# alibaba-damo-academy/Inferix

Hardware: AMD Instinct MI355X
Metric: latent_frames_per_sec (higher is better)
Workload: dtype bf16; 1 GPU; Self-Forcing 480p bf16 (Wan2.1-T2V-1.3B causal DiT, 30 layers), block_size=3, 21 latent frames = 7 blocks x (4 denoise + 1 context) generator forwards, KV prefix 4680..32760 keys in the KV manager's cache (identity page map; page-table form: `streaming_steady`); `value` counts the generator calls (SURVEY 8d), the per-block VAE decode of config 2 is measured beside it under --full (`per_block_decod; batch=1, parallelism=single, layers=30, pair_forwards=True, pair_mode=streams

## Files before the change

### inferix_amd/csrc/ifx_attn.h

```cpp
#pragma once
#include "ifx_common.h"

#ifndef PP_TRACE
#define PP_TRACE 0
#endif
#ifndef PP_PD
#define PP_PD 2
#endif
#ifndef PP_DUAL_FR
#define PP_DUAL_FR 6
#endif

namespace ifx {

namespace pp {
constexpr int KT = 64;
constexpr int HD = 128;
constexpr int PD = PP_PD;
constexpr int RK = PD + 1, RV = PD + 2;
constexpr int K_OFF = 0;
constexpr int LDS_BYTES = (RK + RV) * 16384;
constexpr int LDS_SWP = 8 * 16384;
constexpr int LDS_ALLOC = PP_TRACE ? LDS_SWP + 24576 : (LDS_BYTES > LDS_SWP ? LDS_BYTES : LDS_SWP);
constexpr int LDS_DUAL = 5 * 16384;

constexpr int FR_PLAIN = 0;
constexpr int FR_FREE = 1;
constexpr int FR_SWP = 2;
constexpr int FR_SWP_DUAL = 3;
constexpr int FR_U4 = 5;
constexpr int FR_U6_DUAL = 6;
constexpr int FR_U4_PRE = 7;
constexpr int FR_U6_DUAL_PRE = 8;
}

__device__ __forceinline__ float attn_max3(float a, float b, float c) {
  float r;
  asm("v_max3_f32 %0, %1, %2, %3" : "=v"(r) : "v"(a), "v"(b), "v"(c));
  return r;
}
__device__ __forceinline__ float attn_half_max(float x) {
  float a = x, b = x, r;
  asm volatile("s_nop 1\n\tv_permlane32_swap_b32 %0, %1\n\ts_nop 1\n\tv_max_f32 %2, %0, %1" : "+v"(a), "+v"(b), "=v"(r));
  return r;
}

struct AttnArgsPP {
  const unsigned short* q;
  unsigned short* out;
  float* lse;
  const unsigned short* k;
  const unsigned short* v;
  KvAddr ka;
  int q_rows, heads, kv_start, kv_len, num_slots, q_tiles, per_xcd, total;
  int ldq, ldo;
  float scale, scale_log2;
  int splits, chunk_tiles;
  int kv_heads, q_per_kv;
  float* part_o;
  float* part_lse;
  int n_ranges;
  int rq0[8], rq1[8], rk0[8], rk1[8], rt0[9];
  unsigned ps_magic;
  unsigned* dbg_rescales;
};

struct AttnSchedule {
  int variant;
  int ng;
  int fr, fr_pre;
  int qt;
  int slots;
  int lds_bytes;
  bool pipelined() const { return fr >= pp::FR_SWP; }
};
constexpr AttnSchedule kAttnSchedules[6] = {
// ... 6 lines not shown
};
inline const AttnSchedule& attn_schedule(int variant) { return kAttnSchedules[variant - 2]; }

inline int attn_pick_variant(int variant, int q_rows, int heads) {
  if (variant >= 2 && variant <= 7) return variant;
  if (variant == 0 && q_rows > 0) {
    const int t256 = (q_rows + 255) / 256, t128 = (q_rows + 127) / 128;
    const float u256 = (float)q_rows / (256.f * t256), u128 = (float)q_rows / (128.f * t128);
    if (u128 > 1.1f * u256) return 6;
    if (heads > 0 && t256 * heads > 256) {
      const float c5 = (float)((t256 * heads + 255) / 256);
      const float c6 = (float)((t128 * heads + 511) / 512) / 0.953f;
      if (c6 < 0.95f * c5) return 6;
    }
  }
  return 7;
}

struct AttnLaunch {
  const unsigned short* q = nullptr;
  unsigned short* out = nullptr;
  float* lse = nullptr;
  const ifx_kv_view* kv = nullptr;
  int q_rows = 0, heads = 0;
  int ldq = 0, ldo = 0;
  int kv_start = 0, kv_len = 0;
  float scale = 0.f;
  int splits = 1;
  void* workspace = nullptr;
  int slot_base = 0, slot_cap = 0, *slots_used = nullptr;
  int n_ranges = 0;
  const int *q_ranges = nullptr, *k_ranges = nullptr;
};
int attn_plan(const AttnLaunch& L, int variant, AttnArgsPP& a, int& schedule, int& paged);
int launch_attn_pp(const AttnArgsPP& a, const AttnSchedule& s, int paged, bool write_partials, bool pre, dim3 grid,
                   hipStream_t stream);
int launch_attn_merge(const float* workspace, int slot_cap, int slots_used, unsigned short* out, float* lse, int q_rows,
                      int heads, hipStream_t stream, int ldo = 0);
size_t attn_pp_workspace_bytes(int q_rows, int heads, int splits);
int attn_pp_split_heuristic(int q_rows, int heads, int nkeys, int qt, int slots);

}
```

### inferix_amd/csrc/ifx_attn.hip

```cpp
#include <stdlib.h>
#include <type_traits>

#include "ifx_attn.h"

namespace ifx {

constexpr int QT = 128;
constexpr int KT = 64;
constexpr int HD = 128;

struct AttnArgs {
  const unsigned short* q;
  unsigned short* out;
  float* lse;
  const unsigned short* k;
  const unsigned short* v;
  KvAddr ka;
  int q_rows, heads, kv_start, kv_len, q_tiles, per_xcd, total;
  int ldq, ldo;
  float last_key_bias;
  int kv_heads, q_per_kv;
  float scale, scale_log2;
};

// ... 263 lines not shown
    }
  }
}

size_t attn_pp_workspace_bytes(int q_rows, int heads, int splits) {
  return splits <= 1 ? 0 : (size_t)splits * q_rows * heads * (128 + 1) * sizeof(float);
}

int attn_pp_split_heuristic(int q_rows, int heads, int nkeys, int qt, int slots) {
  const int tiles = ((q_rows + qt - 1) / qt) * heads;
  const int nt = (nkeys + pp::KT - 1) / pp::KT;
  if (tiles * 16 >= slots * 13 || nt < 16) return 1;
  int best = 1;
  float best_eff = (float)tiles / ((float)slots * ((tiles + slots - 1) / slots));
  static float base = -1.f;
  if (base < 0.f) {
    const char* e = getenv("IFX_ATTN_SPLIT_PENALTY");
    base = e ? (float)atof(e) : 0.01f;
  }
  const float part_mb = (float)q_rows * (float)heads * 516.f / 3.6e6f;
  const float pen = base * (part_mb > 1.f ? part_mb : 1.f);
  for (int s = 2; s <= 32 && s * 8 <= nt; ++s) {
    const int wg = tiles * s, rounds = (wg + slots - 1) / slots;
    const float eff = (float)wg / ((float)slots * rounds) * (1.f - pen * s);
    if (eff > best_eff + 1e-3f) best_eff = eff, best = s;
  }
  return best;
}

static KvAddr attn_kv_addr(const ifx_kv_view* kv) {
  return KvAddr{kv->page_table, kv->page_size, kv->page_table ? 0 : kv->seg_split, kv->page_table ? 0 : kv->seg_delta};
}

int attn_plan(const AttnLaunch& L, int variant, AttnArgsPP& a, int& schedule, int& paged) {
  const ifx_kv_view* kv = L.kv;
  const unsigned ps_magic = (kv->page_table && kv->page_size >= 2 && (long long)kv->num_slots * kv->page_size < (1ll << 32))
                                ? (unsigned)((1ull << 32) / (unsigned)kv->page_size) + 1u : 0u;
  paged = 0;
  if (kv->page_table != nullptr) paged = (kv->page_size >= 3 && ps_magic != 0) ? 1 : 2;
  else if (kv->seg_split > 0) paged = 1;
  int kv_start = L.kv_start, kv_len = L.kv_len, rows = L.q_rows, streams = L.heads;
  if (L.n_ranges > 0) {
    kv_start = 0x7fffffff, kv_len = 0, rows = 0;
    for (int i = 0; i < L.n_ranges; ++i) {
      kv_start = min(kv_start, L.k_ranges[2 * i]);
      kv_len = max(kv_len, L.k_ranges[2 * i + 1]);
      rows += L.q_ranges[2 * i + 1] - L.q_ranges[2 * i];
    }
    rows /= L.n_ranges;
    streams = L.heads * L.n_ranges;
  }
  schedule = attn_pick_variant(variant, rows, streams);
  if (L.n_ranges > 0 && !attn_schedule(schedule).pipelined()) schedule = 7;
  if (paged == 2) schedule = 2;
  const int QT = attn_schedule(schedule).qt;
  const bool partial = L.slot_cap > 0;
  a.q = L.q;
  a.out = partial ? nullptr : L.out;
  a.lse = L.lse;
  a.k = kv->k;
  a.v = kv->v;
  a.ka = attn_kv_addr(kv);
  a.q_rows = L.q_rows;
  a.heads = L.heads;
  a.ldq = L.ldq > 0 ? L.ldq : L.heads * 128;
  a.ldo = L.ldo > 0 ? L.ldo : L.heads * 128;
  a.kv_start = kv_start;
// ... 9 lines not shown
    const int* kr = L.k_ranges;
    int order[8];
    for (int i = 0; i < L.n_ranges; ++i) order[i] = i;
    for (int i = 1; i < L.n_ranges; ++i)
      for (int j = i; j > 0 && kr[2 * order[j] + 1] - kr[2 * order[j]] > kr[2 * order[j - 1] + 1] - kr[2 * order[j - 1]]; --j) {
        const int t = order[j];
        order[j] = order[j - 1];
        order[j - 1] = t;
      }
    a.rt0[0] = 0;
    for (int i = 0; i < L.n_ranges; ++i) {
      const int r = order[i];
      a.rq0[i] = L.q_ranges[2 * r], a.rq1[i] = L.q_ranges[2 * r + 1], a.rk0[i] = kr[2 * r], a.rk1[i] = kr[2 * r + 1];
      a.rt0[i + 1] = a.rt0[i] + (a.rq1[i] - a.rq0[i] + QT - 1) / QT;
    }
    a.q_tiles = a.rt0[L.n_ranges];
  }
  const int nt = (kv_len - kv_start + KT - 1) / KT;
  const int splits = max(1, min(L.n_ranges > 0 ? 1 : L.splits, nt));
  a.chunk_tiles = (nt + splits - 1) / splits;
  a.splits = (nt + a.chunk_tiles - 1) / a.chunk_tiles;
  if (partial && L.slot_base + a.splits > L.slot_cap) {
    set_error("ifx_attn_fwd_partial: slots [%d, %d) exceed the workspace's %d", L.slot_base, L.slot_base + a.splits, L.slot_cap);
    return IFX_EINVAL;
  }
  const int cap = partial ? L.slot_cap : a.splits;
  float* ws = (float*)L.workspace;
  a.part_o = ws ? ws + (size_t)L.slot_base * L.q_rows * L.heads * 128 : nullptr;
  a.part_lse = ws ? ws + (size_t)cap * L.q_rows * L.heads * 128 + (size_t)L.slot_base * L.heads * L.q_rows : nullptr;
  a.total = a.q_tiles * L.heads * a.splits;
  a.per_xcd = (a.total + 7) / 8;
  a.scale = L.scale > 0.f ? L.scale : 0.08838834764831845f;
  a.scale_log2 = a.scale * 1.4426950408889634f;
  if ((partial || a.splits > 1) && L.workspace == nullptr) {
    set_error("ifx_attn_fwd_paged_split: split / partial launches need a workspace");
    return IFX_EINVAL;
  }
  return IFX_OK;
}

}

using namespace ifx;

static int attn_check_view(const char* fn, const ifx_kv_view* kv, int heads,
                           const char* heads_text = "%s: heads %d is not a multiple of kv_heads %d") {
  IFX_REQUIRE(kv->head_dim == HD, "%s: head_dim %d not built (128 only)", fn, kv->head_dim);
  IFX_REQUIRE(heads > 0 && kv->kv_heads > 0 && heads % kv->kv_heads == 0, heads_text, fn, heads, kv->kv_heads);
  return IFX_OK;
}

static int attn_launch(const AttnLaunch& L, int variant, void* stream) {
  AttnArgsPP a;
  int schedule, paged;
  if (const int rc = attn_plan(L, variant, a, schedule, paged)) return rc;
  if (L.slots_used) *L.slots_used = a.splits;
  return launch_attn_pp(a, attn_schedule(schedule), paged, a.splits > 1 || L.slot_cap > 0, fabsf(a.scale_log2 - 1.0f) <= 2.5e-7f,
                        dim3(a.per_xcd * 8), (hipStream_t)stream);
}

static int attn_dispatch(const ifx_bf16* q, ifx_bf16* out, float* lse, const ifx_kv_view* kv, int32_t q_rows,
                         int32_t heads, int32_t kv_start, int32_t kv_len, float scale, int32_t splits, void* workspace,
                         int64_t workspace_bytes, void* stream, int32_t ldq = 0, int32_t ldo = 0, int32_t last_key_multiplicity = 1) {
  IFX_REQUIRE(q && out && kv && kv->k && kv->v, "ifx_attn_fwd_paged: null argument");
  if (ldq <= 0) ldq = heads * HD;
  if (ldo <= 0) ldo = heads * HD;
  IFX_REQUIRE(ldq >= heads * HD && ldo >= heads * HD && ldq % 8 == 0 && ldo % 8 == 0,
              "ifx_attn_fwd_paged: row strides (%d, %d) must be >= heads * 128 and multiples of 8", ldq, ldo);
  if (const int rc = attn_check_view("ifx_attn_fwd_paged", kv, heads)) return rc;
  IFX_REQUIRE(q_rows >= 0 && kv_start >= 0 && kv_len > kv_start && kv_len <= kv->num_slots,
              "ifx_attn_fwd_paged: key range [%d, %d) out of range (capacity %d)", kv_start, kv_len, kv->num_slots);
  IFX_REQUIRE(!kv->page_table || kv->page_size > 0, "ifx_attn_fwd_paged: page_size must be > 0");
  if (q_rows == 0) return IFX_OK;
  const int variant = attn_variant();
  if (last_key_multiplicity > 1) {
    IFX_REQUIRE(splits <= 1 && kv_len - kv_start <= 1024 && lse == nullptr,
                "ifx_attn_fwd_dedup: the multiplicity form is built for short key ranges (<= 1024 keys), unsplit, without LSE");
  }
  if (splits > 1)
    IFX_REQUIRE(workspace && workspace_bytes >= (int64_t)attn_pp_workspace_bytes(q_rows, heads, splits),
                "ifx_attn_fwd_paged_split: workspace of %lld B too small for %d splits (need %lld B)",
                (long long)workspace_bytes, splits, (long long)attn_pp_workspace_bytes(q_rows, heads, splits));
  if (splits > 1 || (last_key_multiplicity <= 1 && (variant >= 2 || (variant == 0 && q_rows >= 1024 && kv_len - kv_start > 1024)))) {
    AttnLaunch L;
    L.q = q, L.out = out, L.lse = lse, L.kv = kv;
    L.q_rows = q_rows, L.heads = heads, L.ldq = ldq, L.ldo = ldo;
    L.kv_start = kv_start, L.kv_len = kv_len, L.scale = scale;
    L.splits = splits > 1 ? splits : 1;
    L.workspace = splits > 1 ? workspace : nullptr;
    return attn_launch(L, variant, stream);
  }
// ... 137 lines not shown
```

### inferix_amd/csrc/ifx_attn_pp.hip

```cpp
#include <stdlib.h>
#include <type_traits>

#include "ifx_attn.h"
#include "ifx_launch.h"
#include "ifx_lds_dma.h"

#ifndef PP_ABLATE
#define PP_ABLATE 0
#endif
#ifndef PP_PACKED
#define PP_PACKED 1
#endif
#ifndef PP_PRIO
#define PP_PRIO 2
#endif
#ifndef PP_RING
#define PP_RING 6
#endif
#ifndef PP_SWP_RING
#define PP_SWP_RING 4
#endif
#ifndef PP_SWP_BALANCE
#define PP_SWP_BALANCE 1
#endif
// ... 13 lines not shown
namespace ifx {

typedef float pp_f32x2 __attribute__((ext_vector_type(2)));

__device__ __forceinline__ void pp_wait_tiles(int tiles) {
  if (tiles <= 0) asm volatile("s_waitcnt vmcnt(0)" ::: "memory");
  else if (tiles == 1) asm volatile("s_waitcnt vmcnt(4)" ::: "memory");
  else if (tiles == 2) asm volatile("s_waitcnt vmcnt(8)" ::: "memory");
  else if (tiles == 3) asm volatile("s_waitcnt vmcnt(12)" ::: "memory");
  else asm volatile("s_waitcnt vmcnt(16)" ::: "memory");
}

__device__ __forceinline__ void pp_page_range(const KvAddr& ka, unsigned ps_magic, int kk, int& lo, int& hi, int& off) {
  if (ka.pt == nullptr) {
    const bool up = ka.seg_split > 0 && kk >= ka.seg_split;
    lo = up ? ka.seg_split : 0;
    hi = (up || ka.seg_split <= 0) ? 0x7fffffff : ka.seg_split;
    off = up ? ka.seg_delta : 0;
    return;
  }
  const int pg = (int)__umulhi((unsigned)kk, ps_magic);
  int entry;
  asm volatile("s_load_dword %0, %1, %2\n\ts_waitcnt lgkmcnt(0)" : "=s"(entry) : "s"(ka.pt), "s"(pg * 4) : "memory");
  lo = pg * ka.ps;
  hi = lo + ka.ps;
  off = entry * ka.ps - lo;
}

template <int PAGED, bool SPLIT, int NG, int FR = 0>
__global__ __launch_bounds__(NG * 256, NG == 1 ? 2 : 1) void attn_fwd_pp_kernel(AttnArgsPP A) {
  using namespace pp;
  constexpr int QT = 128 * NG;
  extern __shared__ __attribute__((aligned(16))) unsigned char smem[];
  constexpr bool SWP = FR >= FR_SWP, DUAL = FR == FR_SWP_DUAL || FR == FR_U6_DUAL || FR == FR_U6_DUAL_PRE, U4 = FR == FR_U4 || FR == FR_U4_PRE,
                 U6 = FR == FR_U6_DUAL || FR == FR_U6_DUAL_PRE, CS = U4 || U6;
  constexpr bool PRE = FR == FR_U4_PRE || FR == FR_U6_DUAL_PRE;
  constexpr int PD = (FR == FR_SWP || U4) ? 3 : pp::PD, RK = DUAL ? 2 : (U4 ? 4 : (FR == FR_SWP ? 3 : pp::RK)),
                RV = DUAL ? 3 : (U4 ? 4 : (FR == FR_SWP ? 5 : pp::RV));
  constexpr int K_OFF = CS ? RV * 16384 : 0, V_OFF = CS ? 0 : RK * 16384;
  const int tid = threadIdx.x, lane = tid & 63;
  const int wave = __builtin_amdgcn_readfirstlane(tid >> 6);
  const int grp = (NG == 2 && PP_GROUP) ? (wave & 1) : (wave >> 2);
  const bool loader = wave < 8;
  const int hi = lane >> 5, l31 = lane & 31;

  const int xcd = blockIdx.x & 7, slot_i = blockIdx.x >> 3;
  const int wi = (!SPLIT && A.n_ranges > 0) ? (int)blockIdx.x : xcd * A.per_xcd + slot_i;
  if ((A.n_ranges == 0 && slot_i >= A.per_xcd) || wi >= A.total) return;
  int head, qt, sp = 0;
  if (SPLIT) {
    const int per_head = A.splits * A.q_tiles;
    head = wi / per_head;
    const int rem = wi - head * per_head;
    sp = rem / A.q_tiles;
    qt = rem - sp * A.q_tiles;
  } else if (A.n_ranges > 0) {
    qt = wi / A.heads;
    head = wi - qt * A.heads;
  } else {
    head = wi / A.q_tiles;
    qt = wi - head * A.q_tiles;
  }
  int kv_s = SPLIT ? A.kv_start + sp * A.chunk_tiles * KT : A.kv_start;
  int kv_e = SPLIT ? min(A.kv_len, kv_s + A.chunk_tiles * KT) : A.kv_len;
  int q_base = qt * QT, q_lim = A.q_rows;
  if (!SPLIT && A.n_ranges > 0) {
    int r = 0;
#pragma unroll
    for (int i = 1; i < 8; ++i)
      if (i < A.n_ranges && qt >= A.rt0[i]) r = i;
    q_base = A.rq0[r] + (qt - A.rt0[r]) * QT;
    q_lim = A.rq1[r];
    kv_s = A.rk0[r];
    kv_e = A.rk1[r];
  }
  const int row_stride = A.heads * HD;

  const int qrow = q_base + wave * 32 + l31;
  const int qrow_c = min(qrow, q_lim - 1);
  bf16x8 qf[8];
  {
    const unsigned short* qp = A.q + (size_t)qrow_c * A.ldq + head * HD + hi * 8;
#pragma unroll
    for (int ks = 0; ks < 8; ++ks) qf[ks] = *reinterpret_cast<const bf16x8*>(qp + ks * 16);
  }
  __builtin_amdgcn_s_waitcnt(0x0F70);
  const int row_bytes = A.kv_heads * HD * 2;
  const int kvh = head / A.q_per_kv;
  const int nkeys = kv_e - kv_s;
  const int NT = (nkeys + KT - 1) / KT;
  const unsigned valid_rows = PAGED ? (unsigned)A.num_slots : (unsigned)kv_e;
  const unsigned nrec = (valid_rows - 1) * (unsigned)row_bytes + 256u;
  const v4i krs = make_rsrc(A.k + kvh * HD, nrec);
  const v4i vrs = make_rsrc(A.v + kvh * HD, nrec);
  const unsigned lds00 = (unsigned)(unsigned long long)(lds_ptr_t)smem;
  const int last_key = kv_e - 1;
  int pc_lo = 0, pc_hi = 0, pc_off = 0;
  int lane_pack;
  {
    const int ln0 = __builtin_amdgcn_mbcnt_hi(~0u, __builtin_amdgcn_mbcnt_lo(~0u, 0u));
    const int pc0 = ln0 & 15, row0 = wave * 4 + (ln0 >> 4);
    lane_pack = (ln0 >> 4) * row_bytes + ((pc0 ^ (row0 & 15)) << 4) +
                (int)((unsigned)((((pc0 >> 2) ^ (row0 & 3)) << 2) | (pc0 & 3)) << 28);
  }
  auto issue_w = [&](int t, int wv, int what = 3) {
    unsigned lds0 = lds00 + wv * 1024;
    asm volatile("" : "+s"(lds0));
    int ln = 0;
    if constexpr (PAGED != 0) {
      ln = __builtin_amdgcn_mbcnt_hi(~0u, __builtin_amdgcn_mbcnt_lo(~0u, 0u));
      asm volatile("" : "+v"(ln));
    }
    int lp = lane_pack;
    asm volatile("" : "+v"(lp));
// ... 22 lines not shown
      } else {
#pragma unroll
        for (int r = 0; r < 2; ++r) {
          const int key0 = key00 + 32 * r;
          const int kk = min(key0, last_key);
          if (kk < pc_lo || kk >= pc_hi) pp_page_range(A.ka, A.ps_magic, kk, pc_lo, pc_hi, pc_off);
          int soff = (kk + pc_off) * row_bytes;
          int adj = 0;
          if (kk + 3 > last_key || kk + 3 >= pc_hi) {
            const int j = min(ln >> 4, last_key - kk);
            adj += ((ln >> 4) - j) * row_bytes;
            if (kk + min(3, last_key - kk) >= pc_hi) {
              int lo2, hi2, off2;
              pp_page_range(A.ka, A.ps_magic, pc_hi, lo2, hi2, off2);
              adj -= (kk + ((kk + j >= pc_hi) ? off2 : pc_off)) * row_bytes;
              soff = 0;
            }
          }
          if (what & 1) dma16(krs, kb + r * 8192, k_lane - adj, soff);
          if (what & 2) dma16(vrs, vb + r * 8192, v_lane - adj, soff);
        }
      }
    } else {
#pragma unroll
      for (int r = 0; r < 2; ++r) {
        const int key = min(kv_s + t * KT + wv * 4 + (ln >> 4) + 32 * r, last_key);
        const int delta = (A.ka.slot(key) - (ln >> 4)) * row_bytes;
        if (what & 1) dma16(krs, kb + r * 8192, k_lane + delta, 0);
        if (what & 2) dma16(vrs, vb + r * 8192, v_lane + delta, 0);
      }
    }
  };
  auto issue = [&](int t) { issue_w(t, wave); };

  f32x16 o[4];
#pragma unroll
  for (int d = 0; d < 4; ++d)
#pragma unroll
    for (int r = 0; r < 16; ++r) o[d][r] = 0.f;
  float m_run = -INFINITY, l_run = 0.f;
  const float c2 = PRE ? 1.0f : A.scale_log2;
  const int kswz = l31 & 15;
  const int vi = lane & 15, vg1 = (lane >> 4) & 1;
  const int v_rowq = vi >> 2;
  const int v_in = (vg1 << 5) | ((vi & 3) << 3);

  f32x16 s[2];
  bf16x8 pb[2][2];
  bf16x8 fA[4], fB[4];
  constexpr int RD = FR == FR_FREE ? PP_RING : 3, LA = RD - 1;
  bf16x8 fr[RD][2];
  pb[0][0] = pb[0][1] = pb[1][0] = pb[1][1] = bf16x8{};
  if (PP_ABLATE) {
#pragma unroll
    for (int i = 0; i < 4; ++i) fA[i] = fB[i] = bf16x8{};
    pb[0][0] = pb[0][1] = pb[1][0] = pb[1][1] = bf16x8{};
    s[0] = s[1] = f32x16{};
  }

  auto ldV = [&](bf16x8(&f)[4], const unsigned char* vb, int b, int s2) {
    if (PP_ABLATE & 4) return;
    const unsigned char* vr0 = vb + (32 * b + 16 * s2 + 4 * hi + v_rowq) * 256 + v_in;
    const unsigned char* vr1 = vr0 + 8 * 256;
#pragma unroll
    for (int d = 0; d < 4; ++d) {
      const int ch = (d ^ v_rowq) << 6;
// ... 746 lines not shown
        for (int e = 0; e < 4; ++e) acc[e] += w * v[u][e];
      }
    }
  }
  const float inv = 1.0f / den;
  u16x4 w4;
#pragma unroll
  for (int e = 0; e < 4; ++e) w4[e] = f2bf(acc[e] * inv);
  *reinterpret_cast<u16x4*>(out + (size_t)row * ldo + head * 128 + c) = w4;
  if (lse != nullptr && c == 0) lse[(size_t)head * q_rows + row] = mx + __logf(den);
}

template <int NG, int FR>
static int launch_pp(const AttnArgsPP& a, int paged, bool split, dim3 grid, int lds, hipStream_t stream) {
  auto launch = [&](auto kind) {
    constexpr int P = decltype(kind)::value;
    const char* const what = "ifx_attn_fwd_paged(pp)";
    return split ? launch_lds<attn_fwd_pp_kernel<P, true, NG, FR>>(grid, dim3(NG * 256), lds, stream, what, a)
                 : launch_lds<attn_fwd_pp_kernel<P, false, NG, FR>>(grid, dim3(NG * 256), lds, stream, what, a);
  };
  if constexpr (NG == 2 && FR == pp::FR_PLAIN) {
    if (paged == 2) return launch(std::integral_constant<int, 2>{});
  }
  return paged ? launch(std::integral_constant<int, 1>{}) : launch(std::integral_constant<int, 0>{});
}

static void launch_merge(const float* part_o, const float* part_lse, unsigned short* out, float* lse, int q_rows, int heads, int splits,
                         int ldo, hipStream_t stream) {
  const int pairs = q_rows * heads;
  hipLaunchKernelGGL(attn_split_merge_kernel, dim3((pairs + 7) / 8), dim3(256), 0, stream, part_o, part_lse, out, lse, q_rows, heads,
                     splits, ldo);
}

int launch_attn_pp(const AttnArgsPP& a, const AttnSchedule& s, int paged, bool write_partials, bool pre, dim3 grid, hipStream_t stream) {
  using namespace pp;
  const AttnSchedule& own = attn_schedule(s.variant);
  const int fr = pre ? own.fr_pre : own.fr;
  if (paged == 2 && !(own.ng == 2 && fr == FR_PLAIN)) {
    set_error("ifx_attn_fwd_paged(pp): per-lane page translation is built for the plain two-group schedule only (not variant %d)", s.variant);
    return IFX_EUNSUP;
  }
#define PP_CASE(NG, FR) \
  case (NG) * 16 + (FR): rc = launch_pp<NG, FR>(a, paged, write_partials, grid, own.lds_bytes, stream); break
  int rc = IFX_OK;
  switch (own.ng * 16 + fr) {
    PP_CASE(1, FR_U6_DUAL_PRE);
    PP_CASE(1, PP_DUAL_FR);
    PP_CASE(2, FR_SWP);
    PP_CASE(2, FR_U4_PRE);
    PP_CASE(2, FR_U4);
    PP_CASE(2, FR_FREE);
    PP_CASE(3, FR_PLAIN);
    PP_CASE(2, FR_PLAIN);
    default:
      set_error("ifx_attn_fwd_paged(pp): no kernel built for %d wave groups in loop form %d", own.ng, fr);
      return IFX_EUNSUP;
  }
#undef PP_CASE
  if (rc != IFX_OK) return rc;
  if (a.splits > 1 && a.out != nullptr) launch_merge(a.part_o, a.part_lse, a.out, a.lse, a.q_rows, a.heads, a.splits, a.ldo, stream);
  return check_launch("ifx_attn_fwd_paged(pp)");
}

int launch_attn_merge(const float* workspace, int slot_cap, int slots_used, unsigned short* out, float* lse, int q_rows,
                      int heads, hipStream_t stream, int ldo) {
  launch_merge(workspace, workspace + (size_t)slot_cap * q_rows * heads * 128, out, lse, q_rows, heads, slots_used,
               ldo > 0 ? ldo : heads * 128, stream);
  return check_launch("ifx_attn_merge_partials");
}

}
```

### inferix_amd/csrc/ifx_common.h

```cpp
#pragma once
#include <hip/hip_runtime.h>
#include <stdint.h>
#include <stdio.h>
#include <stdlib.h>

#include "../../include/inferix_hip.h"

namespace ifx {

constexpr int kWave = 64;

typedef __attribute__((ext_vector_type(8))) __bf16 bf16x8;
typedef __attribute__((ext_vector_type(4))) __bf16 bf16x4;
typedef __attribute__((ext_vector_type(8))) unsigned short u16x8;
typedef __attribute__((ext_vector_type(4))) unsigned short u16x4;
typedef __attribute__((ext_vector_type(4))) short s16x4;
typedef __attribute__((ext_vector_type(4))) float f32x4;
typedef __attribute__((ext_vector_type(16))) float f32x16;
typedef __attribute__((ext_vector_type(4))) unsigned int u32x4;
typedef __attribute__((ext_vector_type(2))) unsigned int u32x2;

__device__ __forceinline__ float bf2f(unsigned short u) {
  return __builtin_bit_cast(float, (unsigned int)u << 16);
}
// ... 62 lines not shown
}
__device__ __forceinline__ float wave_max(float v) {
  v = fmaxf(v, dpp_or<0xB1, 0xf>(v, v));
  v = fmaxf(v, dpp_or<0x4E, 0xf>(v, v));
  v = fmaxf(v, dpp_or<0x141, 0xf>(v, v));
  v = fmaxf(v, dpp_or<0x140, 0xf>(v, v));
  v = fmaxf(v, dpp_or<0x142, 0xa>(v, v));
  v = fmaxf(v, dpp_or<0x143, 0xc>(v, v));
  return __builtin_bit_cast(float, __builtin_amdgcn_readlane(__builtin_bit_cast(int, v), 63));
}

struct KvAddr {
  const int32_t* pt;
  int32_t ps;
  int32_t seg_split, seg_delta;
  __device__ __forceinline__ int slot(int t) const {
    if (pt == nullptr) return (seg_split > 0 && t >= seg_split) ? t + seg_delta : t;
    int pg = t / ps;
    return pt[pg] * ps + (t - pg * ps);
  }
};

void set_error(const char* fmt, ...);
int check_launch(const char* what);
int gemm_variant();
int gemm_small_split();
unsigned* device_error_word();
long long spin_timeout_ticks();
int spin_fault();
int gemm_pp_variant();
int conv_variant();
unsigned* attn_debug_counter();
int attn_variant();
static inline int lab_env_int(const char* name, int dflt) {
  const char* e = getenv(name);
  return e ? atoi(e) : dflt;
}

}

#define IFX_REQUIRE(cond, ...)            \
  do {                                    \
    if (!(cond)) {                        \
      ifx::set_error(__VA_ARGS__);        \
      return IFX_EINVAL;                  \
    }                                     \
  } while (0)
```

### inferix_amd/csrc/ifx_core.hip

```cpp
#include <stdarg.h>
#include <stdlib.h>
#include <string.h>

#include <atomic>

#include "ifx_common.h"

namespace ifx {
static thread_local char g_err[512] = "";

void set_error(const char* fmt, ...) {
  va_list ap;
  va_start(ap, fmt);
  vsnprintf(g_err, sizeof(g_err), fmt, ap);
  va_end(ap);
}

static std::atomic<int> g_gemm_variant{-1}, g_gemm_pp_variant{-1}, g_attn_variant{-1}, g_conv_variant{-1}, g_spin_timeout_ms{-1}, g_spin_fault{0};
static thread_local int g_gemm_small_split = -1;
static int opt_get(const std::atomic<int>& slot) { return slot.load(std::memory_order_relaxed); }
static int opt_get(int slot) { return slot; }
static void opt_set(std::atomic<int>& slot, int v) { slot.store(v, std::memory_order_relaxed); }
static void opt_set(int& slot, int v) { slot = v; }
template <class Slot>
static int opt_or_env(Slot& slot, const char* env, int dflt = 0) {
  int v = opt_get(slot);
  if (v < 0) {
    const char* e = getenv(env);
    opt_set(slot, v = e ? atoi(e) : dflt);
  }
  return v;
}
int gemm_variant() { return opt_or_env(g_gemm_variant, "IFX_GEMM_VARIANT"); }
int gemm_pp_variant() { return opt_or_env(g_gemm_pp_variant, "IFX_GEMM_PP_VARIANT"); }
int attn_variant() { return opt_or_env(g_attn_variant, "IFX_ATTN_VARIANT"); }
int conv_variant() { return opt_or_env(g_conv_variant, "IFX_CONV_VARIANT"); }
static unsigned* g_attn_dbg = nullptr;
static bool g_attn_dbg_on = false;
unsigned* attn_debug_counter() { return g_attn_dbg_on ? g_attn_dbg : nullptr; }
int gemm_small_split() { return opt_or_env(g_gemm_small_split, "IFX_GEMM_SMALL_SPLIT"); }

static std::atomic<unsigned*> g_dev_err{nullptr};
unsigned* device_error_word() {
  static unsigned* const word = [] {
    void* p = nullptr;
    if (hipHostMalloc(&p, 64, hipHostMallocMapped | hipHostMallocPortable) != hipSuccess || p == nullptr) return (unsigned*)nullptr;
    memset(p, 0, 64);
    g_dev_err.store((unsigned*)p, std::memory_order_release);
    return (unsigned*)p;
  }();
  return word;
}
long long spin_timeout_ticks() { return (long long)max(1, opt_or_env(g_spin_timeout_ms, "IFX_SPIN_TIMEOUT_MS", 2000)) * 100000LL; }
int spin_fault() { return opt_get(g_spin_fault); }
static thread_local char g_err_dev[640] = "";

int check_launch(const char* what) {
  hipError_t e = hipGetLastError();
  if (e != hipSuccess) {
    set_error("%s: launch failed: %s", what, hipGetErrorString(e));
    return IFX_ELAUNCH;
  }
  return IFX_OK;
}
}

extern "C" int ifx_version(void) { return (0 << 16) | (IFX_ABI_MINOR << 8) | 0; }
extern "C" int32_t ifx_device_error(int32_t clear) {
  unsigned* w = ifx::g_dev_err.load(std::memory_order_acquire);
  if (w == nullptr) return 0;
  const unsigned v = __atomic_load_n(w, __ATOMIC_ACQUIRE);
  if (v != 0 && clear) __atomic_store_n(w, 0u, __ATOMIC_RELEASE);
  return (int32_t)v;
}
extern "C" const char* ifx_last_error(void) {
  const unsigned v = (unsigned)ifx_device_error(1);
  if (v == 0) return ifx::g_err;
  const unsigned kind = v >> 24, detail = v & 0xffffffu;
  snprintf(ifx::g_err_dev, sizeof(ifx::g_err_dev),
           "device: a kernel gave up a wait (%s, flag %u) after the spin budget — the producing workgroup was not resident or did not "
           "finish; the results of that launch are invalid%s%s",
           kind == 1 ? "split-K / stream-K consumer of ifx_gemm_bf16_ws / ifx_gemm_q8_ws" : "unknown waiter", detail,
           ifx::g_err[0] ? "; last host error: " : "", ifx::g_err);
  return ifx::g_err_dev;
}
extern "C" const char* ifx_arch(void) { return "gfx950"; }
extern "C" int ifx_set_option(const char* key, int32_t value) {
  if (key && !strcmp(key, "gemm_variant") && value >= 0 && value <= 29) { ifx::opt_set(ifx::g_gemm_variant, value); return IFX_OK; }
  if (key && !strcmp(key, "gemm_small_split") && (value == 0 || value == 1)) { ifx::opt_set(ifx::g_gemm_small_split, value); return IFX_OK; }
  if (key && !strcmp(key, "attn_variant") && value >= 0 && value <= 7) { ifx::opt_set(ifx::g_attn_variant, value); return IFX_OK; }
  if (key && !strcmp(key, "conv_variant") && value >= 0 && value <= 1) { ifx::opt_set(ifx::g_conv_variant, value); return IFX_OK; }
  if (key && !strcmp(key, "gemm_pp_variant") && value >= 0 && value <= 1) { ifx::opt_set(ifx::g_gemm_pp_variant, value); return IFX_OK; }
  if (key && !strcmp(key, "attn_debug_counters") && (value == 0 || value == 1)) {
    if (value == 1) {
      if (ifx::g_attn_dbg == nullptr && hipMalloc((void**)&ifx::g_attn_dbg, 64) != hipSuccess) {
        ifx::g_attn_dbg = nullptr;
        ifx::set_error("ifx_set_option: attn_debug_counters: hipMalloc failed");
        return IFX_ELAUNCH;
      }
      (void)hipDeviceSynchronize();
      (void)hipMemset(ifx::g_attn_dbg, 0, 64);
    }
    ifx::g_attn_dbg_on = value == 1;
    return IFX_OK;
  }
  if (key && !strcmp(key, "spin_timeout_ms") && value >= 1 && value <= 600000) { ifx::opt_set(ifx::g_spin_timeout_ms, value); return IFX_OK; }
  if (key && !strcmp(key, "spin_fault") && (value == 0 || value == 1)) { ifx::opt_set(ifx::g_spin_fault, value); return IFX_OK; }
  ifx::set_error("ifx_set_option: unknown key or value out of range: %s = %d", key ? key : "(null)", (int)value);
  return IFX_EINVAL;
}
extern "C" int ifx_get_option(const char* key, int32_t* value) {
  if (key == nullptr || value == nullptr) { ifx::set_error("ifx_get_option: null argument"); return IFX_EINVAL; }
  if (!strcmp(key, "gemm_variant")) { *value = ifx::gemm_variant(); return IFX_OK; }
  if (!strcmp(key, "gemm_small_split")) { *value = ifx::gemm_small_split(); return IFX_OK; }
  if (!strcmp(key, "attn_variant")) { *value = ifx::attn_variant(); return IFX_OK; }
  if (!strcmp(key, "conv_variant")) { *value = ifx::conv_variant(); return IFX_OK; }
  if (!strcmp(key, "gemm_pp_variant")) { *value = ifx::gemm_pp_variant(); return IFX_OK; }
  if (!strcmp(key, "attn_debug_counters")) { *value = ifx::g_attn_dbg_on ? 1 : 0; return IFX_OK; }
  if (!strcmp(key, "attn_rescale_count")) {
    unsigned v = 0;
    if (ifx::g_attn_dbg != nullptr) {
      (void)hipDeviceSynchronize();
      (void)hipMemcpy(&v, ifx::g_attn_dbg, sizeof(v), hipMemcpyDeviceToHost);
    }
    *value = (int32_t)(v & 0x7fffffffu);
    return IFX_OK;
  }
  if (!strcmp(key, "spin_timeout_ms")) { *value = (int32_t)(ifx::spin_timeout_ticks() / 100000LL); return IFX_OK; }
  if (!strcmp(key, "spin_fault")) { *value = ifx::spin_fault(); return IFX_OK; }
  ifx::set_error("ifx_get_option: unknown key: %s", key);
  return IFX_EINVAL;
}
```

Baseline: 22.73 frames/s.

## Add 16x16x32 MFMA form of the variant-7 attention loop for long KV prefixes

Adds a new attention inner-loop form that uses 16x16x32 bf16 MFMA instructions, with each wave handling two 16-row query blocks, instead of the 32x32 layout. It has its own swizzled K/V LDS addressing, transposed V reads, a quad-level row max, and an interleaved exp/MFMA schedule. By default it is picked only for variant 7 with prescaled softmax, no split, and at least 14040 keys, and an option or environment variable can force it on or off. The aim is better MFMA throughput and overlap of the softmax with the matrix math on long prefixes, at the cost of a large new code path and possible changes in register pressure.

```diff
diff --git a/inferix_amd/csrc/ifx_attn.h b/inferix_amd/csrc/ifx_attn.h
--- a/inferix_amd/csrc/ifx_attn.h
+++ b/inferix_amd/csrc/ifx_attn.h
@@ -32,6 +32,8 @@
 constexpr int FR_U6_DUAL = 6;
 constexpr int FR_U4_PRE = 7;
 constexpr int FR_U6_DUAL_PRE = 8;
+constexpr int FR_U4_M16 = 9;
+constexpr int FR_U4_PRE_M16 = 10;
 }
 
 __device__ __forceinline__ float attn_max3(float a, float b, float c) {
@@ -42,6 +44,13 @@
 __device__ __forceinline__ float attn_half_max(float x) {
   float a = x, b = x, r;
   asm volatile("s_nop 1\n\tv_permlane32_swap_b32 %0, %1\n\ts_nop 1\n\tv_max_f32 %2, %0, %1" : "+v"(a), "+v"(b), "=v"(r));
+  return r;
+}
+
+__device__ __forceinline__ float attn_quad_max(float x) {
+  const float h = attn_half_max(x);
+  float a = h, b = h, r;
+  asm volatile("s_nop 1\n\tv_permlane16_swap_b32 %0, %1\n\ts_nop 1\n\tv_max_f32 %2, %0, %1" : "+v"(a), "+v"(b), "=v"(r));
   return r;
 }
 
@@ -114,8 +123,16 @@
   int n_ranges = 0;
   const int *q_ranges = nullptr, *k_ranges = nullptr;
 };
-int attn_plan(const AttnLaunch& L, int variant, AttnArgsPP& a, int& schedule, int& paged);
-int launch_attn_pp(const AttnArgsPP& a, const AttnSchedule& s, int paged, bool write_partials, bool pre, dim3 grid,
+struct AttnForm {
+  bool pre = false, mfma16 = false;
+};
+inline bool attn_pick_mfma16(int mfma, int schedule, bool pre, bool split, int nkeys) {
+  if (schedule != 7 || mfma == 1) return false;
+  if (mfma == 2) return true;
+  return pre && !split && nkeys >= 14040;
+}
+int attn_plan(const AttnLaunch& L, int variant, int mfma, AttnArgsPP& a, int& schedule, int& paged, AttnForm& form);
+int launch_attn_pp(const AttnArgsPP& a, const AttnSchedule& s, int paged, bool write_partials, AttnForm form, dim3 grid,
                    hipStream_t stream);
 int launch_attn_merge(const float* workspace, int slot_cap, int slots_used, unsigned short* out, float* lse, int q_rows,
                       int heads, hipStream_t stream, int ldo = 0);
diff --git a/inferix_amd/csrc/ifx_attn.hip b/inferix_amd/csrc/ifx_attn.hip
--- a/inferix_amd/csrc/ifx_attn.hip
+++ b/inferix_amd/csrc/ifx_attn.hip
@@ -319,7 +319,7 @@
   return KvAddr{kv->page_table, kv->page_size, kv->page_table ? 0 : kv->seg_split, kv->page_table ? 0 : kv->seg_delta};
 }
 
-int attn_plan(const AttnLaunch& L, int variant, AttnArgsPP& a, int& schedule, int& paged) {
+int attn_plan(const AttnLaunch& L, int variant, int mfma, AttnArgsPP& a, int& schedule, int& paged, AttnForm& form) {
   const ifx_kv_view* kv = L.kv;
   const unsigned ps_magic = (kv->page_table && kv->page_size >= 2 && (long long)kv->num_slots * kv->page_size < (1ll << 32))
                                 ? (unsigned)((1ull << 32) / (unsigned)kv->page_size) + 1u : 0u;
@@ -395,6 +395,8 @@
   a.per_xcd = (a.total + 7) / 8;
   a.scale = L.scale > 0.f ? L.scale : 0.08838834764831845f;
   a.scale_log2 = a.scale * 1.4426950408889634f;
+  form.pre = fabsf(a.scale_log2 - 1.0f) <= 2.5e-7f;
+  form.mfma16 = attn_pick_mfma16(mfma, schedule, form.pre, partial || a.splits > 1, kv_len - kv_start);
   if ((partial || a.splits > 1) && L.workspace == nullptr) {
     set_error("ifx_attn_fwd_paged_split: split / partial launches need a workspace");
     return IFX_EINVAL;
@@ -416,10 +418,10 @@
 static int attn_launch(const AttnLaunch& L, int variant, void* stream) {
   AttnArgsPP a;
   int schedule, paged;
-  if (const int rc = attn_plan(L, variant, a, schedule, paged)) return rc;
+  AttnForm form;
+  if (const int rc = attn_plan(L, variant, attn_mfma(), a, schedule, paged, form)) return rc;
   if (L.slots_used) *L.slots_used = a.splits;
-  return launch_attn_pp(a, attn_schedule(schedule), paged, a.splits > 1 || L.slot_cap > 0, fabsf(a.scale_log2 - 1.0f) <= 2.5e-7f,
-                        dim3(a.per_xcd * 8), (hipStream_t)stream);
+  return launch_attn_pp(a, attn_schedule(schedule), paged, a.splits > 1 || L.slot_cap > 0, form, dim3(a.per_xcd * 8), (hipStream_t)stream);
 }
 
 static int attn_dispatch(const ifx_bf16* q, ifx_bf16* out, float* lse, const ifx_kv_view* kv, int32_t q_rows,
diff --git a/inferix_amd/csrc/ifx_attn_pp.hip b/inferix_amd/csrc/ifx_attn_pp.hip
--- a/inferix_amd/csrc/ifx_attn_pp.hip
+++ b/inferix_amd/csrc/ifx_attn_pp.hip
@@ -69,9 +69,10 @@
   using namespace pp;
   constexpr int QT = 128 * NG;
   extern __shared__ __attribute__((aligned(16))) unsigned char smem[];
-  constexpr bool SWP = FR >= FR_SWP, DUAL = FR == FR_SWP_DUAL || FR == FR_U6_DUAL || FR == FR_U6_DUAL_PRE, U4 = FR == FR_U4 || FR == FR_U4_PRE,
+  constexpr bool M16 = FR == FR_U4_M16 || FR == FR_U4_PRE_M16;
+  constexpr bool SWP = FR >= FR_SWP, DUAL = FR == FR_SWP_DUAL || FR == FR_U6_DUAL || FR == FR_U6_DUAL_PRE, U4 = FR == FR_U4 || FR == FR_U4_PRE || M16,
                  U6 = FR == FR_U6_DUAL || FR == FR_U6_DUAL_PRE, CS = U4 || U6;
-  constexpr bool PRE = FR == FR_U4_PRE || FR == FR_U6_DUAL_PRE;
+  constexpr bool PRE = FR == FR_U4_PRE || FR == FR_U6_DUAL_PRE || FR == FR_U4_PRE_M16;
   constexpr int PD = (FR == FR_SWP || U4) ? 3 : pp::PD, RK = DUAL ? 2 : (U4 ? 4 : (FR == FR_SWP ? 3 : pp::RK)),
                 RV = DUAL ? 3 : (U4 ? 4 : (FR == FR_SWP ? 5 : pp::RV));
   constexpr int K_OFF = CS ? RV * 16384 : 0, V_OFF = CS ? 0 : RK * 16384;
@@ -116,7 +117,15 @@
   const int qrow = q_base + wave * 32 + l31;
   const int qrow_c = min(qrow, q_lim - 1);
   bf16x8 qf[8];
-  {
+  if constexpr (M16) {
+#pragma unroll
+    for (int qb = 0; qb < 2; ++qb) {
+      const int qr = min(q_base + wave * 32 + 16 * qb + (lane & 15), q_lim - 1);
+      const unsigned short* qp = A.q + (size_t)qr * A.ldq + head * HD + (lane >> 4) * 8;
+#pragma unroll
+      for (int st = 0; st < 4; ++st) qf[4 * qb + st] = *reinterpret_cast<const bf16x8*>(qp + st * 32);
+    }
+  } else {
     const unsigned short* qp = A.q + (size_t)qrow_c * A.ldq + head * HD + hi * 8;
 #pragma unroll
     for (int ks = 0; ks < 8; ++ks) qf[ks] = *reinterpret_cast<const bf16x8*>(qp + ks * 16);
@@ -205,6 +214,287 @@
     }
   };
   auto issue = [&](int t) { issue_w(t, wave); };
+
+  if constexpr (M16) {
+    const int g16 = lane >> 4, i16 = lane & 15;
+    f32x4 o[8][2];
+#pragma unroll
+    for (int db = 0; db < 8; ++db) o[db][0] = o[db][1] = f32x4{0.f, 0.f, 0.f, 0.f};
+    float m_run[2] = {-INFINITY, -INFINITY}, l_run[2] = {0.f, 0.f};
+    const float c2 = PRE ? 1.0f : A.scale_log2;
+    f32x4 sA[4][2], sB[4][2];
+    bf16x8 pA[2][2], pB[2][2];
+    pA[0][0] = pA[0][1] = pA[1][0] = pA[1][1] = bf16x8{};
+    pB[0][0] = pB[0][1] = pB[1][0] = pB[1][1] = bf16x8{};
+    f32x4 negm[2];
+    auto set_negm = [&](int qb, float m) {
+      negm[qb] = f32x4{-m, -m, -m, -m};
+      asm volatile("" : "+v"(negm[qb]));
+    };
+    if (PRE) {
+      set_negm(0, 0.f);
+      set_negm(1, 0.f);
+    }
+    int kterm[4], vterm[4];
+#pragma unroll
+    for (int st = 0; st < 4; ++st) {
+      kterm[st] = K_OFF + i16 * 256 + (((4 * st + g16) ^ i16) << 4);
+      asm volatile("" : "+v"(kterm[st]));
+    }
+#pragma unroll
+    for (int c = 0; c < 4; ++c) {
+      vterm[c] = (4 * g16 + (i16 >> 2)) * 256 + ((c ^ (i16 >> 2)) << 6) + ((i16 & 3) << 3);
+      asm volatile("" : "+v"(vterm[c]));
+    }
+    auto mfma16 = [](const bf16x8& a, const bf16x8& b, const f32x4& c) { return __builtin_amdgcn_mfma_f32_16x16x32_bf16(a, b, c, 0, 0, 0); };
+    auto ld_v = [&](int vbase, int ks, int db) -> bf16x8 {
+      const unsigned char* a0 = smem + vterm[db >> 1] + (vbase + 32 * ks * 256 + (db & 1) * 32);
+      const bf16x4 t0 = __builtin_amdgcn_ds_read_tr16_b64_v4bf16((bf16x4 __attribute__((address_space(3)))*)(a0));
+      const bf16x4 t1 = __builtin_amdgcn_ds_read_tr16_b64_v4bf16((bf16x4 __attribute__((address_space(3)))*)(a0 + 4096));
+      return __builtin_shufflevector(t0, t1, 0, 1, 2, 3, 4, 5, 6, 7);
+    };
+    auto ld_k = [&](int kbase, int kb, int st) -> bf16x8 {
+      return *reinterpret_cast<const bf16x8*>(smem + kterm[st] + (kbase + 16 * kb * 256));
+    };
+    auto mask_ragged = [&](int t, f32x4(&sx)[4][2]) {
+      int kidx = t * KT + 4 * g16;
+      asm volatile("" : "+v"(kidx));
+#pragma unroll
+      for (int kb = 0; kb < 4; ++kb)
+#pragma unroll
+        for (int qb = 0; qb < 2; ++qb)
+#pragma unroll
+          for (int r = 0; r < 4; ++r)
+            if (kidx + 16 * kb + r >= nkeys) sx[kb][qb][r] = -INFINITY;
+    };
+    auto true_max = [&](f32x4(&sx)[4][2], int qb, float floor_v) -> float {
+      float mx = attn_max3(__builtin_fmaxf(sx[0][qb][0], sx[1][qb][0]), floor_v, floor_v);
+#pragma unroll
+      for (int r = 1; r < 4; ++r) mx = attn_max3(mx, sx[0][qb][r], sx[1][qb][r]);
+#pragma unroll
+      for (int r = 0; r < 4; ++r) mx = attn_max3(mx, sx[2][qb][r], sx[3][qb][r]);
+      return attn_quad_max(mx);
+    };
+    auto exp_plain = [&](f32x4(&sx)[4][2], bf16x8(&px)[2][2], int qb, float mc) -> float {
+      float a0 = 0.f, a1 = 0.f;
+#pragma unroll
+      for (int kb = 0; kb < 4; ++kb)
+#pragma unroll
+        for (int r = 0; r < 4; r += 2) {
+          const float p0 = __builtin_amdgcn_exp2f(sx[kb][qb][r] * c2 - mc);
+          const float p1 = __builtin_amdgcn_exp2f(sx[kb][qb][r + 1] * c2 - mc);
+          a0 += p0;
+          a1 += p1;
+          px[kb >> 1][qb][4 * (kb & 1) + r] = static_cast<__bf16>(p0);
+          px[kb >> 1][qb][4 * (kb & 1) + r + 1] = static_cast<__bf16>(p1);
+        }
+      return a0 + a1;
+    };
+    auto rescale_o = [&](int qb, float alpha) {
+#pragma unroll
+      for (int db = 0; db < 8; ++db) o[db][qb] *= alpha;
+    };
+    auto body = [&](f32x4(&sC)[4][2], f32x4(&sN)[4][2], bf16x8(&pC)[2][2], bf16x8(&pP)[2][2], auto kslot_c, auto vslot_c, float(&tsum)[2]) {
+      constexpr int KSLOT = decltype(kslot_c)::value, VSLOT = decltype(vslot_c)::value;
+      constexpr int RDs = PRE ? 2 : PP_SWP_RING, LAs = RDs - 1;
+      bf16x8 fs[RDs][2];
+      auto load = [&](int j) {
+        bf16x8(&f)[2] = fs[j % RDs];
+        if (j < 8) {
+#pragma unroll
+          for (int e = 0; e < 2; ++e) f[e] = ld_v(VSLOT * 16384, j >> 2, 2 * (j & 3) + e);
+        } else {
+          const int q = j - 8;
+#pragma unroll
+          for (int e = 0; e < 2; ++e) f[e] = ld_k(KSLOT * 16384, q >> 1, 2 * (q & 1) + e);
+        }
+      };
+      auto mma1 = [&](int j, int e, int qb) {
+        const bf16x8& f = fs[j % RDs][e];
+        if (j < 8) {
+          const int ks = j >> 2, db = 2 * (j & 3) + e;
+          o[db][qb] = mfma16(f, pP[ks][qb], o[db][qb]);
+        } else {
+          const int q = j - 8, kb = q >> 1, st = 2 * (q & 1) + e;
+          if (st == 0) sN[kb][qb] = mfma16(f, qf[4 * qb + st], PRE ? negm[qb] : f32x4{0.f, 0.f, 0.f, 0.f});
+          else sN[kb][qb] = mfma16(f, qf[4 * qb + st], sN[kb][qb]);
+        }
+      };
+      float p0 = 0.f, p1 = 0.f, e1 = 0.f;
+      float acc4[4] = {0.f, 0.f, 0.f, 0.f};
+      u32x4 pw[2][2];
+      const float mc[2] = {m_run[0] * c2, m_run[1] * c2};
+#pragma unroll
+      for (int j = 0; j < LAs; ++j) load(j);
+#pragma unroll
+      for (int j = 0; j < 16; ++j) {
+        const int ks = j >> 3, qb = (j >> 2) & 1, w = j & 3, kb = 2 * ks + (w >> 1), r0 = 2 * (w & 1);
+        __builtin_amdgcn_sched_barrier(0);
+        if (j + LAs < 16) load(j + LAs);
+        mma1(j, 0, 0);
+        if (PRE) {
+          p0 = __builtin_amdgcn_exp2f(sC[kb][qb][r0]);
+          e1 = sC[kb][qb][r0 + 1];
+        } else {
+          p0 = __builtin_amdgcn_exp2f(__builtin_fmaf(sC[kb][qb][r0], c2, -mc[qb]));
+          e1 = __builtin_fmaf(sC[kb][qb][r0 + 1], c2, -mc[qb]);
+          asm volatile("" : "+v"(e1));
+        }
+        mma1(j, 0, 1);
+        __builtin_amdgcn_sched_barrier(0);
+        mma1(j, 1, 0);
+        p1 = __builtin_amdgcn_exp2f(e1);
+        mma1(j, 1, 1);
+        asm volatile("s_nop 0\n\tv_add_f32 %0, %0, %1" : "+v"(acc4[2 * qb]) : "v"(p0));
+        asm volatile("v_add_f32 %0, %0, %1" : "+v"(acc4[2 * qb + 1]) : "v"(p1));
+        unsigned pk;
+        asm volatile("v_cvt_pk_bf16_f32 %0, %1, %2" : "=v"(pk) : "v"(p0), "v"(p1));
+        pw[ks][qb][w] = pk;
+      }
+      __builtin_amdgcn_sched_barrier(0);
+#pragma unroll
+      for (int ks = 0; ks < 2; ++ks)
+#pragma unroll
+        for (int qb = 0; qb < 2; ++qb) pC[ks][qb] = __builtin_bit_cast(bf16x8, pw[ks][qb]);
+      tsum[0] = acc4[0] + acc4[1];
+      tsum[1] = acc4[2] + acc4[3];
+    };
+    auto iteration = [&](int t, f32x4(&sC)[4][2], f32x4(&sN)[4][2], bf16x8(&pC)[2][2], bf16x8(&pP)[2][2], auto kslot_c, auto vslot_c) {
+      if (t + 2 < NT) asm volatile("s_waitcnt vmcnt(8)" ::: "memory");
+      else asm volatile("s_waitcnt vmcnt(0)" ::: "memory");
+      asm volatile("s_waitcnt lgkmcnt(0)" ::: "memory");
+      __builtin_amdgcn_s_barrier();
+      if (wave < 4) {
+        if (t + 3 < NT) {
+          issue_w(t + 3, wave, 1);
+          issue_w(t + 3, wave + 4, 1);
+        }
+        if (t + 2 < NT) {
+          issue_w(t + 2, wave, 2);
+          issue_w(t + 2, wave + 4, 2);
+        }
+      }
+      if (t == NT - 1 && (nkeys & (KT - 1))) mask_ragged(t, sC);
+      float tsum[2];
+      body(sC, sN, pC, pP, kslot_c, vslot_c, tsum);
+      if (__any(!(tsum[0] < 1048576.f) || !(tsum[1] < 1048576.f))) {
+        if (A.dbg_rescales != nullptr && lane == 0) atomicAdd(A.dbg_rescales, 1u);
+#pragma unroll
+        for (int qb = 0; qb < 2; ++qb) {
+          if (PRE) {
+            const float d = true_max(sC, qb, 0.f);
+            const float alpha = __builtin_amdgcn_exp2f(-d);
+            tsum[qb] = exp_plain(sC, pC, qb, d);
+            m_run[qb] += d;
+            l_run[qb] *= alpha;
+            rescale_o(qb, alpha);
+            set_negm(qb, m_run[qb]);
+#pragma unroll
+            for (int kb = 0; kb < 4; ++kb)
+#pragma unroll
+              for (int r = 0; r < 4; ++r) sN[kb][qb][r] -= d;
+          } else {
+            const float m_new = true_max(sC, qb, m_run[qb]);
+            const float alpha = __builtin_amdgcn_exp2f((m_run[qb] - m_new) * c2);
+            m_run[qb] = m_new;
+            tsum[qb] = exp_plain(sC, pC, qb, m_new * c2);
+            l_run[qb] *= alpha;
+            rescale_o(qb, alpha);
+          }
+        }
+      }
+      l_run[0] += tsum[0];
+      l_run[1] += tsum[1];
+    };
+    *reinterpret_cast<u32x4*>(smem + V_OFF + 3 * 16384 + tid * 32) = u32x4{0, 0, 0, 0};
+    *reinterpret_cast<u32x4*>(smem + V_OFF + 3 * 16384 + tid * 32 + 16) = u32x4{0, 0, 0, 0};
+    if (wave < 4) {
+      issue_w(0, wave, 3);
+      issue_w(0, wave + 4, 3);
+      if (NT > 1) {
+        issue_w(1, wave, 3);
+        issue_w(1, wave + 4, 3);
+      }
+      if (NT > 2) {
+        issue_w(2, wave, 1);
+        issue_w(2, wave + 4, 1);
+        asm volatile("s_waitcnt vmcnt(4)" ::: "memory");
+      } else {
+        asm volatile("s_waitcnt vmcnt(0)" ::: "memory");
+      }
+    }
+    asm volatile("s_waitcnt lgkmcnt(0)" ::: "memory");
+    __builtin_amdgcn_s_barrier();
+#pragma unroll
+    for (int kb = 0; kb < 4; ++kb)
+#pragma unroll
+      for (int qb = 0; qb < 2; ++qb) {
+        sA[kb][qb] = f32x4{0.f, 0.f, 0.f, 0.f};
+#pragma unroll
+        for (int st = 0; st < 4; ++st) sA[kb][qb] = mfma16(ld_k(0, kb, st), qf[4 * qb + st], sA[kb][qb]);
+      }
+    if (NT == 1 && (nkeys & (KT - 1))) mask_ragged(0, sA);
+#pragma unroll
+    for (int qb = 0; qb < 2; ++qb) {
+      m_run[qb] = true_max(sA, qb, m_run[qb]);
+      if (PRE) {
+        set_negm(qb, m_run[qb]);
+#pragma unroll
+        for (int kb = 0; kb < 4; ++kb)
+#pragma unroll
+          for (int r = 0; r < 4; ++r) sA[kb][qb][r] -= m_run[qb];
+      }
+    }
+    for (int t = 0; t < NT; t += 4) {
+      iteration(t, sA, sB, pA, pB, std::integral_constant<int, 1>{}, std::integral_constant<int, 3>{});
+      if (t + 1 < NT) iteration(t + 1, sB, sA, pB, pA, std::integral_constant<int, 2>{}, std::integral_constant<int, 0>{});
+      if (t + 2 < NT) iteration(t + 2, sA, sB, pA, pB, std::integral_constant<int, 3>{}, std::integral_constant<int, 1>{});
+      if (t + 3 < NT) iteration(t + 3, sB, sA, pB, pA, std::integral_constant<int, 0>{}, std::integral_constant<int, 2>{});
+    }
+    if (!(NT & 1)) {
+      pA[0][0] = pB[0][0];
+      pA[0][1] = pB[0][1];
+      pA[1][0] = pB[1][0];
+      pA[1][1] = pB[1][1];
+    }
+    {
+      const int vbase = V_OFF + ((NT - 1) % RV) * 16384;
+#pragma unroll
+      for (int ks = 0; ks < 2; ++ks)
+#pragma unroll
+        for (int db = 0; db < 8; ++db) {
+          const bf16x8 f = ld_v(vbase, ks, db);
+          o[db][0] = mfma16(f, pA[ks][0], o[db][0]);
+          o[db][1] = mfma16(f, pA[ks][1], o[db][1]);
+        }
+    }
+#pragma unroll
+    for (int qb = 0; qb < 2; ++qb) {
+      float l_tot = l_run[qb] + __shfl_xor(l_run[qb], 16, 64);
+      l_tot += __shfl_xor(l_tot, 32, 64);
+      const float inv = 1.0f / l_tot;
+      const int qr = q_base + wave * 32 + 16 * qb + i16;
+      if (SPLIT) {
+        if (qr < A.q_rows) {
+          float* op = A.part_o + ((size_t)sp * A.q_rows + qr) * row_stride + head * HD + 4 * g16;
+#pragma unroll
+          for (int db = 0; db < 8; ++db) *reinterpret_cast<f32x4*>(op + 16 * db) = o[db][qb] * inv;
+          if (g16 == 0) A.part_lse[((size_t)sp * A.heads + head) * A.q_rows + qr] = m_run[qb] * A.scale + __logf(l_tot);
+        }
+      } else if (qr < q_lim) {
+        unsigned short* op = A.out + (size_t)qr * A.ldo + head * HD + 4 * g16;
+#pragma unroll
+        for (int db = 0; db < 8; ++db) {
+          u16x4 w4;
+#pragma unroll
+          for (int e = 0; e < 4; ++e) w4[e] = f2bf(o[db][qb][e] * inv);
+          *reinterpret_cast<u16x4*>(op + 16 * db) = w4;
+        }
+        if (A.lse != nullptr && g16 == 0) A.lse[(size_t)head * A.q_rows + qr] = m_run[qb] * A.scale + __logf(l_tot);
+      }
+    }
+    return;
+  }
 
   f32x16 o[4];
 #pragma unroll
@@ -1017,10 +1307,17 @@
                      splits, ldo);
 }
 
-int launch_attn_pp(const AttnArgsPP& a, const AttnSchedule& s, int paged, bool write_partials, bool pre, dim3 grid, hipStream_t stream) {
+int launch_attn_pp(const AttnArgsPP& a, const AttnSchedule& s, int paged, bool write_partials, AttnForm form, dim3 grid, hipStream_t stream) {
   using namespace pp;
   const AttnSchedule& own = attn_schedule(s.variant);
-  const int fr = pre ? own.fr_pre : own.fr;
+  int fr = form.pre ? own.fr_pre : own.fr;
+  if (form.mfma16) {
+    if (fr != FR_U4 && fr != FR_U4_PRE) {
+      set_error("ifx_attn_fwd_paged(pp): the 16x16x32 form is built for the constant-slot loop of variant 7 only (not variant %d)", s.variant);
+      return IFX_EUNSUP;
+    }
+    fr = fr == FR_U4 ? FR_U4_M16 : FR_U4_PRE_M16;
+  }
   if (paged == 2 && !(own.ng == 2 && fr == FR_PLAIN)) {
     set_error("ifx_attn_fwd_paged(pp): per-lane page translation is built for the plain two-group schedule only (not variant %d)", s.variant);
     return IFX_EUNSUP;
@@ -1034,6 +1331,8 @@
     PP_CASE(2, FR_SWP);
     PP_CASE(2, FR_U4_PRE);
     PP_CASE(2, FR_U4);
+    PP_CASE(2, FR_U4_PRE_M16);
+    PP_CASE(2, FR_U4_M16);
     PP_CASE(2, FR_FREE);
     PP_CASE(3, FR_PLAIN);
     PP_CASE(2, FR_PLAIN);
diff --git a/inferix_amd/csrc/ifx_common.h b/inferix_amd/csrc/ifx_common.h
--- a/inferix_amd/csrc/ifx_common.h
+++ b/inferix_amd/csrc/ifx_common.h
@@ -118,6 +118,7 @@
 int conv_variant();
 unsigned* attn_debug_counter();
 int attn_variant();
+int attn_mfma();
 static inline int lab_env_int(const char* name, int dflt) {
   const char* e = getenv(name);
   return e ? atoi(e) : dflt;
diff --git a/inferix_amd/csrc/ifx_core.hip b/inferix_amd/csrc/ifx_core.hip
--- a/inferix_amd/csrc/ifx_core.hip
+++ b/inferix_amd/csrc/ifx_core.hip
@@ -16,7 +16,7 @@
   va_end(ap);
 }
 
-static std::atomic<int> g_gemm_variant{-1}, g_gemm_pp_variant{-1}, g_attn_variant{-1}, g_conv_variant{-1}, g_spin_timeout_ms{-1}, g_spin_fault{0};
+static std::atomic<int> g_gemm_variant{-1}, g_gemm_pp_variant{-1}, g_attn_variant{-1}, g_attn_mfma{-1}, g_conv_variant{-1}, g_spin_timeout_ms{-1}, g_spin_fault{0};
 static thread_local int g_gemm_small_split = -1;
 static int opt_get(const std::atomic<int>& slot) { return slot.load(std::memory_order_relaxed); }
 static int opt_get(int slot) { return slot; }
@@ -34,6 +34,7 @@
 int gemm_variant() { return opt_or_env(g_gemm_variant, "IFX_GEMM_VARIANT"); }
 int gemm_pp_variant() { return opt_or_env(g_gemm_pp_variant, "IFX_GEMM_PP_VARIANT"); }
 int attn_variant() { return opt_or_env(g_attn_variant, "IFX_ATTN_VARIANT"); }
+int attn_mfma() { return opt_or_env(g_attn_mfma, "IFX_ATTN_MFMA"); }
 int conv_variant() { return opt_or_env(g_conv_variant, "IFX_CONV_VARIANT"); }
 static unsigned* g_attn_dbg = nullptr;
 static bool g_attn_dbg_on = false;
@@ -89,6 +90,7 @@
   if (key && !strcmp(key, "gemm_variant") && value >= 0 && value <= 29) { ifx::opt_set(ifx::g_gemm_variant, value); return IFX_OK; }
   if (key && !strcmp(key, "gemm_small_split") && (value == 0 || value == 1)) { ifx::opt_set(ifx::g_gemm_small_split, value); return IFX_OK; }
   if (key && !strcmp(key, "attn_variant") && value >= 0 && value <= 7) { ifx::opt_set(ifx::g_attn_variant, value); return IFX_OK; }
+  if (key && !strcmp(key, "attn_mfma") && value >= 0 && value <= 2) { ifx::opt_set(ifx::g_attn_mfma, value); return IFX_OK; }
   if (key && !strcmp(key, "conv_variant") && value >= 0 && value <= 1) { ifx::opt_set(ifx::g_conv_variant, value); return IFX_OK; }
   if (key && !strcmp(key, "gemm_pp_variant") && value >= 0 && value <= 1) { ifx::opt_set(ifx::g_gemm_pp_variant, value); return IFX_OK; }
   if (key && !strcmp(key, "attn_debug_counters") && (value == 0 || value == 1)) {
@@ -114,6 +116,7 @@
   if (!strcmp(key, "gemm_variant")) { *value = ifx::gemm_variant(); return IFX_OK; }
   if (!strcmp(key, "gemm_small_split")) { *value = ifx::gemm_small_split(); return IFX_OK; }
   if (!strcmp(key, "attn_variant")) { *value = ifx::attn_variant(); return IFX_OK; }
+  if (!strcmp(key, "attn_mfma")) { *value = ifx::attn_mfma(); return IFX_OK; }
   if (!strcmp(key, "conv_variant")) { *value = ifx::conv_variant(); return IFX_OK; }
   if (!strcmp(key, "gemm_pp_variant")) { *value = ifx::gemm_pp_variant(); return IFX_OK; }
   if (!strcmp(key, "attn_debug_counters")) { *value = ifx::g_attn_dbg_on ? 1 : 0; return IFX_OK; }
```

After: 22.99 frames/s (median of 6 runs). 1.1% higher.
